# huj31415/nbody3d-webgpu

Hardware: AMD Instinct MI355X
Metric: pair-interactions/s (higher is better)
Workload: dtype f32; 1 GPU; N=262144 Plummer sphere, dt=1e-3, G=1, eps2=1e-4, i-sharded over 1 GPU(s); n=262144, kernel_variant=f32pk_symw_ipl16_j1_w2048_r32t128, parallelism=1gpu

## Files before the change

nbody3d-webgpu_amd/csrc/kernels/symmetric.hip.h:

```cpp
#pragma once

namespace nb {

template <typename T> struct SymRowT { T x, y, z; };
using SymRow = SymRowT<float>;

constexpr uint32_t kFlushSteps = 4096;

template <int NG>
__device__ __forceinline__ void flush_resident_sums(float (*hi)[64], const int lane, const bool flushed, nb_f2 (&ax)[NG], nb_f2 (&ay)[NG], nb_f2 (&az)[NG])
{
    if (flushed) {
#pragma unroll
        for (int c = 0; c < NG; ++c) {
            hi[6 * c + 0][lane] += ax[c].x; hi[6 * c + 1][lane] += ay[c].x; hi[6 * c + 2][lane] += az[c].x;
            hi[6 * c + 3][lane] += ax[c].y; hi[6 * c + 4][lane] += ay[c].y; hi[6 * c + 5][lane] += az[c].y;
        }
    } else {
#pragma unroll
        for (int c = 0; c < NG; ++c) {
            hi[6 * c + 0][lane] = ax[c].x; hi[6 * c + 1][lane] = ay[c].x; hi[6 * c + 2][lane] = az[c].x;
            hi[6 * c + 3][lane] = ax[c].y; hi[6 * c + 4][lane] = ay[c].y; hi[6 * c + 5][lane] = az[c].y;
        }
    }
// ... 95 lines not shown
                    for (int c = 0; c < 4; ++c) si[c] = pm * r[c];
#pragma unroll
                    for (int c = 0; c < 4; ++c) sj[c] = mi[c0g + c] * r[c];
#pragma unroll
                    for (int c = 0; c < 4; ++c) ax[c0g + c] = __builtin_elementwise_fma(si[c], dx[c], ax[c0g + c]);
#pragma unroll
                    for (int c = 0; c < 4; ++c) ay[c0g + c] = __builtin_elementwise_fma(si[c], dy[c], ay[c0g + c]);
#pragma unroll
                    for (int c = 0; c < 4; ++c) az[c0g + c] = __builtin_elementwise_fma(si[c], dz[c], az[c0g + c]);
#pragma unroll
                    for (int c = 0; c < 4; ++c) bx[u] = __builtin_elementwise_fma(-sj[c], dx[c], bx[u]);
#pragma unroll
                    for (int c = 0; c < 4; ++c) by[u] = __builtin_elementwise_fma(-sj[c], dy[c], by[u]);
#pragma unroll
                    for (int c = 0; c < 4; ++c) bz[u] = __builtin_elementwise_fma(-sj[c], dz[c], bz[u]);
                }
            }
#pragma unroll
            for (int u = 0; u < J; ++u) {
                tx[u] = wave_rot1(tx[u]); ty[u] = wave_rot1(ty[u]); tz[u] = wave_rot1(tz[u]); tm[u] = wave_rot1(tm[u]);
                bx[u] = nb_f2{wave_rot1(bx[u].x), wave_rot1(bx[u].y)};
                by[u] = nb_f2{wave_rot1(by[u].x), wave_rot1(by[u].y)};
                bz[u] = nb_f2{wave_rot1(bz[u].x), wave_rot1(bz[u].y)};
            }
        }
        if (sym) {
            SymRow* out = partial + (size_t)(pl.t_layer0 + d) * pl.np + tstart + lane;
            if constexpr (WS == 1) {
#pragma unroll
                for (int u = 0; u < J; ++u) out[u * 64] = SymRow{bx[u].x + bx[u].y, by[u].x + by[u].y, bz[u].x + bz[u].y};
            } else {
                const int buf = done++ & 1;
#pragma unroll
                for (int u = 0; u < J; ++u) {
                    red[buf][w][3 * u + 0][lane] = bx[u].x + bx[u].y;
                    red[buf][w][3 * u + 1][lane] = by[u].x + by[u].y;
                    red[buf][w][3 * u + 2][lane] = bz[u].x + bz[u].y;
                }
                __syncthreads();
                if (w == done % WS) {
#pragma unroll
                    for (int u = 0; u < J; ++u) {
                        float sx = red[buf][0][3 * u + 0][lane], sy = red[buf][0][3 * u + 1][lane], sz = red[buf][0][3 * u + 2][lane];
#pragma unroll
                        for (int ww = 1; ww < WS; ++ww) { sx += red[buf][ww][3 * u + 0][lane]; sy += red[buf][ww][3 * u + 1][lane]; sz += red[buf][ww][3 * u + 2][lane]; }
                        out[u * 64] = SymRow{sx, sy, sz};
                    }
                }
            }
        }
    }
    SymRow* out = partial + (size_t)(pl.r_layer0 + q) * pl.np + (size_t)g * S + w * RB + lane;
#pragma unroll
    for (int c = 0; c < NG; ++c) {
        out[(2 * c) * 64] = SymRow{ax[c].x, ay[c].x, az[c].x};
        out[(2 * c + 1) * 64] = SymRow{ax[c].y, ay[c].y, az[c].y};
    }
}

struct SymWK { uint32_t np, nsb, W, total_hi, total_lo, n_hi, zc, ups, r_layer0, t_layer0; };
#define SYMW_PLAN_PARAMS const uint32_t W_, const uint32_t ups_, const uint32_t nsb_, const uint32_t zc_, const uint32_t r_layer0_, const uint32_t t_layer0_
typedef uint32_t nb_u4 __attribute__((ext_vector_type(4)));
template <int TAIL>
__device__ __forceinline__ void symw_record_and_tail(const uint32_t* rec_at, nb_u4& rec, uint32_t (&tail)[TAIL])
{
    static_assert(TAIL == 1 || TAIL == 4, "f32: eps2; f64: G, eps2");
    constexpr int kTailOffset = 4 * 8 + 6 * 4;
    if constexpr (TAIL == 1) {
        asm volatile("s_load_dwordx4 %0, %2, 0x0\n\ts_load_dword %1, %3, %4\n\ts_waitcnt lgkmcnt(0)"
                     : "=&s"(rec), "=&s"(tail[0]) : "s"(rec_at), "s"(__builtin_amdgcn_kernarg_segment_ptr()), "n"(kTailOffset) : "memory");
    } else {
        nb_u4 t;
        asm volatile("s_load_dwordx4 %0, %2, 0x0\n\ts_load_dwordx4 %1, %3, %4\n\ts_waitcnt lgkmcnt(0)"
                     : "=&s"(rec), "=&s"(t) : "s"(rec_at), "s"(__builtin_amdgcn_kernarg_segment_ptr()), "n"(kTailOffset) : "memory");
        tail[0] = t.x; tail[1] = t.y; tail[2] = t.z; tail[3] = t.w;
    }
}

__device__ __forceinline__ SymWK symw_plan_words(uint32_t S, uint32_t cps, uint32_t W, uint32_t ups, uint32_t nsb, uint32_t zc, uint32_t r_layer0, uint32_t t_layer0)
{
    const uint32_t H = (nsb - 1u) >> 1, n_hi = (nsb & 1u) ? 0u : nsb >> 1;
    const uint32_t total_lo = (H + 1u) * cps + zc, total_hi = total_lo + (n_hi ? cps : 0u);
    return SymWK{(nsb + (zc ? 1u : 0u)) * S, nsb, W, total_hi, total_lo, n_hi, zc, ups, r_layer0, t_layer0};
}

template <int NG, int J, bool PAIR>
__device__ __forceinline__ void symw_sweeps(const uint32_t* __restrict__ gtab, const float4* __restrict__ bodies, SymRow* __restrict__ partial, SymRow* __restrict__ spill,
                                            SYMW_PLAN_PARAMS, uint32_t* __restrict__ queue, const uint32_t npieces, const uint32_t pieces_off)
{
    static_assert(!PAIR || J == 1, "paired sweeps: one traveler per lane and sweep");
    constexpr uint32_t S = 128u * NG;
    constexpr int GW = NG < 4 ? NG : 4;
    constexpr uint32_t CH = 64u * J;
    constexpr uint32_t CPS = S / CH;
    const SymWK pl = symw_plan_words(S, CPS, W_, ups_, nsb_, zc_, r_layer0_, t_layer0_);
    const int lane = threadIdx.x & 63, wi = threadIdx.x >> 6;
    const uint32_t w = __builtin_amdgcn_readfirstlane(blockIdx.x * 4u + wi);
    const bool active = w < pl.W;
    NB_STAMP(0);
    __shared__ float red[4][6 * NG][64];
    __shared__ uint32_t fin[4];
    const uint32_t ups = pl.ups, ush = (uint32_t)__builtin_ctz(ups), ustep = 64u >> ush,
                   tab1 = 2u * (pl.np / S);
    nb_u4 rec;
    uint32_t tail[1];
    symw_record_and_tail(gtab + tab1 + 4u * (active ? w : 0u), rec, tail);
    const float eps2 = __builtin_bit_cast(float, tail[0]);
    const nb_f2 e2 = nb_f2{eps2, eps2};
    const uint32_t first_lo = pl.n_hi * pl.total_hi, first_z = first_lo + (pl.nsb - pl.n_hi) * pl.total_lo;
    const uint32_t slot = rec.w;
    NB_STAMP_LIGHT(1);
    bool first_part = true;

    auto run = [&](uint32_t u, const uint32_t uend, const uint32_t piece_layer) -> uint32_t {
        uint32_t gfin = ~0u;
        while (u < uend) {
            const uint32_t p = u >> ush;
            uint32_t g, k, total;
            if (p < first_lo) { g = p / pl.total_hi; k = p - g * pl.total_hi; total = pl.total_hi; }
            else if (p < first_z) { const uint32_t r = p - first_lo; g = pl.n_hi + r / pl.total_lo; k = r - (g - pl.n_hi) * pl.total_lo; total = pl.total_lo; }
            else { g = pl.nsb; k = p - first_z; total = pl.zc; }
            const uint32_t ring = g < pl.nsb ? total - CPS - pl.zc : 0u;
            const uint32_t both_end = g < pl.nsb ? ring + pl.zc : 0u;
            uint32_t ug_end = (p - k + total) * ups;
            if (ug_end > uend) ug_end = uend;

            nb_f2 xi[NG], yi[NG], zi[NG], mi[NG], ax[NG], ay[NG], az[NG];
            {
                const float4* rb = bodies + (size_t)g * S + lane;
#pragma unroll
                for (int c = 0; c < NG; ++c) {
                    const float4 b0 = ld4(rb + (2 * c) * 64), b1 = ld4(rb + (2 * c + 1) * 64);
                    xi[c] = nb_f2{b0.x, b1.x}; yi[c] = nb_f2{b0.y, b1.y}; zi[c] = nb_f2{b0.z, b1.z}; mi[c] = nb_f2{b0.w, b1.w};
                    ax[c] = nb_f2{0, 0}; ay[c] = nb_f2{0, 0}; az[c] = nb_f2{0, 0};
                }
            }
            uint32_t since = 0;
            bool flushed = false;
            while (u < ug_end) {
                const uint32_t q0 = u & (ups - 1u);
                bool pair = false;
                if constexpr (PAIR) pair = q0 == 0u && ug_end - u >= 2u * ups && k + 1u < both_end;
                uint32_t nun = ups - q0;
                if (nun > ug_end - u) nun = ug_end - u;
                const uint32_t s0 = q0 * ustep, s1 = s0 + nun * ustep;
                u += pair ? 2u * ups : nun;
                if (since >= kFlushSteps) {
                    flush_resident_sums<NG>(red[wi], lane, flushed, ax, ay, az);
                    flushed = true;
                    since = 0;
                }
                since += pair ? 128u : s1 - s0;
                const bool sym = k < both_end, zsweep = k >= ring && sym;
                const uint32_t d = k / CPS;
                uint32_t tb = g + 1 + d;
                if (tb >= pl.nsb) tb -= pl.nsb;
                const uint32_t tstart = k < ring ? tb * S + (k % CPS) * CH : zsweep ? pl.nsb * S + (k - ring) * CH : g * S + (k - both_end) * CH;
                const uint32_t zrow = g * pl.zc + (k - ring);
                ++k;
                if constexpr (PAIR) {
                    if (pair) {
                        const bool zsweep1 = k >= ring;
                        const uint32_t d1 = k / CPS;
                        uint32_t tb1 = g + 1 + d1;
                        if (tb1 >= pl.nsb) tb1 -= pl.nsb;
                        const uint32_t tstart1 = zsweep1 ? pl.nsb * S + (k - ring) * CH : tb1 * S + (k % CPS) * CH;
// ... 319 lines not shown
                                uu[c] = nb_fma(t3 * e, 1.5, t3);
                            }
#pragma unroll
                            for (int c = 0; c < GW; ++c) {
                                const double si = tm * uu[c];
                                ax[c0g + c] = nb_fma(si, dx[c], ax[c0g + c]); ay[c0g + c] = nb_fma(si, dy[c], ay[c0g + c]); az[c0g + c] = nb_fma(si, dz[c], az[c0g + c]);
                                if constexpr (BOTH) {
                                    const double sj = mi[c0g + c] * uu[c];
                                    bx = nb_fma(-sj, dx[c], bx); by = nb_fma(-sj, dy[c], by); bz = nb_fma(-sj, dz[c], bz);
                                }
                            }
                        }
                        tx = wave_rot1(tx); ty = wave_rot1(ty); tz = wave_rot1(tz); tm = wave_rot1(tm);
                        if constexpr (BOTH) { bx = wave_rot1(bx); by = wave_rot1(by); bz = wave_rot1(bz); }
                    }
                };
                if (sym) steps(std::true_type{}); else steps(std::false_type{});
                if (sym) {
                    SymRowT<double>* out = (s0 != 0 ? spill + (size_t)slot * CH : zsweep ? spill + (size_t)zrow * CH : partial + (size_t)(pl.t_layer0 + d) * pl.np + tstart)
                                           + (((uint32_t)lane - s1) & 63u);
                    *out = SymRowT<double>{bx, by, bz};
                }
            }
            if (u >= uend && piece_layer != ~0u) {
                SymRowT<double>* out = partial + (size_t)(pl.r_layer0 + piece_layer) * pl.np + (size_t)g * S + lane;
#pragma unroll
                for (int c = 0; c < IPL; ++c) out[c * 64] = SymRowT<double>{ax[c], ay[c], az[c]};
                return g;
            }
            if (u >= uend) {
                gfin = g;
#pragma unroll
                for (int c = 0; c < IPL; ++c) { red[wi][3 * c + 0][lane] = ax[c]; red[wi][3 * c + 1][lane] = ay[c]; red[wi][3 * c + 2][lane] = az[c]; }
                break;
            }
            SymRowT<double>* out = partial + (size_t)(pl.r_layer0 + gtab[2 * g + 1] - 1u) * pl.np + (size_t)g * S + lane;
#pragma unroll
            for (int c = 0; c < IPL; ++c) out[c * 64] = SymRowT<double>{ax[c], ay[c], az[c]};
        }
        return gfin;
    };
    const uint32_t gfin = run(active ? rec.x : 0u, active ? rec.y : 0u, ~0u);
    if (lane == 0) fin[wi] = gfin;
    __syncthreads();
    if (gfin != ~0u) {
        int members = 0, mine = 0;
#pragma unroll
        for (int j = 0; j < 4; ++j) {
            const bool same = fin[j] == gfin;
            members += same;
            mine += same && j < wi;
        }
        SymRowT<double>* out = partial + (size_t)(pl.r_layer0 + rec.z) * pl.np + (size_t)gfin * S + lane;
        for (int r = mine; r < IPL; r += members) {
            double sx = 0, sy = 0, sz = 0;
#pragma unroll
            for (int j = 0; j < 4; ++j)
                if (fin[j] == gfin) { sx += red[j][3 * r + 0][lane]; sy += red[j][3 * r + 1][lane]; sz += red[j][3 * r + 2][lane]; }
            out[r * 64] = SymRowT<double>{sx, sy, sz};
        }
    }
    if (npieces) {
        for (;;) {
            uint32_t id = 0;
            if (lane == 0) id = __hip_atomic_fetch_add(queue, 1u, __ATOMIC_RELAXED, __HIP_MEMORY_SCOPE_AGENT);
            id = __builtin_amdgcn_readfirstlane(id);
            if (id >= npieces) break;
            const uint32_t pu = gtab[pieces_off + 2u * id], ll = gtab[pieces_off + 2u * id + 1u];
            (void)run(pu, pu + (ll >> 16), ll & 0xffffu);
        }
    }
}

__device__ __forceinline__ uint32_t rank_find(const uint32_t* __restrict__ prefix, uint32_t ng, uint32_t p)
{
    uint32_t lo = 0, hi = ng;
    while (hi - lo > 1) {
        const uint32_t mid = (lo + hi) >> 1;
        if (prefix[mid] <= p) lo = mid; else hi = mid;
    }
    return lo;
}

template <int NG>
__global__ __launch_bounds__(256) __attribute__((amdgpu_waves_per_eu(NG > 4 ? 2 : 4, NG > 4 ? 2 : 4)))
void nb_force_symw_rank(const float4* __restrict__ bodies, SymRow* __restrict__ partial, const uint32_t* __restrict__ tab, const SymRankPlan pl,
                        const uint32_t n, const float eps2, const uint32_t wave0, const uint32_t wave_end, SymRow* __restrict__ spill,
                        const uint32_t k_lo, const uint32_t k_hi, const uint32_t d0)
{
    constexpr uint32_t S = 128u * NG, CPS = S / 64u;
    constexpr int GW = NG < 4 ? NG : 4;
    const int lane = threadIdx.x & 63;
    const uint32_t w = wave0 + __builtin_amdgcn_readfirstlane(blockIdx.x * 4u + (threadIdx.x >> 6));
    if (w >= wave_end) return;
    const bool phase_b = w >= pl.WA;
    const uint32_t wl = phase_b ? w - pl.WA : w, Lp = phase_b ? pl.LB : pl.LA, Wp = phase_b ? pl.WB : pl.WA;
    const uint32_t ng = pl.g1 - pl.g0;
    const size_t lstride = (size_t)ng * S;
    const uint32_t* __restrict__ prefix = tab + 4 * pl.nsb + (phase_b ? ng + 1 : 0);
    const uint32_t ups = pl.ups, ustep = 64u / ups;
    const uint64_t Lu = (uint64_t)Lp * ups;
    uint32_t u = (uint32_t)(((uint64_t)wl * Lu) / Wp);
    const uint32_t uend = (uint32_t)(((uint64_t)(wl + 1) * Lu) / Wp);
    const nb_f2 e2 = nb_f2{eps2, eps2};
    __shared__ float hi[4][6 * NG][64];
    const int wi = threadIdx.x >> 6;
    while (u < uend) {
        const uint32_t ps = u / ups;
        const uint32_t gi = rank_find(prefix, ng, ps), g = pl.g0 + gi;
        uint32_t j = ps - prefix[gi];
        uint32_t ug_end = prefix[gi + 1] * ups;
        if (ug_end > uend) ug_end = uend;
        const uint32_t total = g < pl.n_hi ? pl.total_hi : pl.total_lo, ring = total - CPS;
        uint32_t a = (pl.g1 - 1 - g) * CPS;
        if (a > ring) a = ring;
        const uint32_t a_lo = a < k_lo ? a : k_lo, a_len = (a < k_hi ? a : k_hi) - a_lo;
        uint32_t b_lo = a > k_lo ? a : k_lo;
        if (b_lo > ring) b_lo = ring;

        nb_f2 xi[NG], yi[NG], zi[NG], mi[NG], ax[NG], ay[NG], az[NG];
        {
            const float4* rb = bodies + (size_t)g * S + lane;
#pragma unroll
            for (int c = 0; c < NG; ++c) {
                const float4 b0 = ld4(rb + (2 * c) * 64), b1 = ld4(rb + (2 * c + 1) * 64);
                xi[c] = nb_f2{b0.x, b1.x}; yi[c] = nb_f2{b0.y, b1.y}; zi[c] = nb_f2{b0.z, b1.z}; mi[c] = nb_f2{b0.w, b1.w};
                ax[c] = nb_f2{0, 0}; ay[c] = nb_f2{0, 0}; az[c] = nb_f2{0, 0};
            }
        }
        uint32_t since = 0;
        bool flushed = false;
        while (u < ug_end) {
            const uint32_t q0 = u % ups;
            uint32_t nun = ups - q0;
            if (nun > ug_end - u) nun = ug_end - u;
            const uint32_t s0 = q0 * ustep, s1 = s0 + nun * ustep;
            u += nun;
            const uint32_t k = phase_b ? b_lo + j : (j < a_len ? a_lo + j : ring + (j - a_len));
            ++j;
            const bool sym = k < ring;
            const uint32_t d = k / CPS;
            uint32_t tb = g + 1 + d;
            if (tb >= pl.nsb) tb -= pl.nsb;
            const uint32_t tstart = sym ? tb * S + (k % CPS) * 64u : g * S + (k - ring) * 64u;
            if (tstart >= n) continue;
            if (since >= kFlushSteps) {
                flush_resident_sums<NG>(hi[wi], lane, flushed, ax, ay, az);
                flushed = true;
                since = 0;
            }
            since += s1 - s0;
            const float4 t = ld4(bodies + tstart + (((uint32_t)lane - s0) & 63u));
            float tx = t.x, ty = t.y, tz = t.z, tm = t.w;
            nb_f2 bx = nb_f2{0, 0}, by = nb_f2{0, 0}, bz = nb_f2{0, 0};
            for (uint32_t st = s0; st < s1; ++st) {
                const nb_f2 px = nb_f2{tx, tx}, py = nb_f2{ty, ty}, pz = nb_f2{tz, tz}, pm = nb_f2{tm, tm};
#pragma unroll
                for (int c0g = 0; c0g < NG; c0g += GW) {
                    nb_f2 dx[GW], dy[GW], dz[GW], d2[GW], r[GW], si[GW], sj[GW];
#pragma unroll
                    for (int c = 0; c < GW; ++c) dx[c] = px - xi[c0g + c];
#pragma unroll
                    for (int c = 0; c < GW; ++c) dy[c] = py - yi[c0g + c];
#pragma unroll
                    for (int c = 0; c < GW; ++c) dz[c] = pz - zi[c0g + c];
#pragma unroll
                    for (int c = 0; c < GW; ++c) d2[c] = __builtin_elementwise_fma(dx[c], dx[c], e2);
#pragma unroll
                    for (int c = 0; c < GW; ++c) d2[c] = __builtin_elementwise_fma(dy[c], dy[c], d2[c]);
#pragma unroll
                    for (int c = 0; c < GW; ++c) d2[c] = __builtin_elementwise_fma(dz[c], dz[c], d2[c]);
#pragma unroll
                    for (int c = 0; c < GW; ++c) r[c] = d2[c] * d2[c];
#pragma unroll
                    for (int c = 0; c < GW; ++c) r[c] = r[c] * d2[c];
#pragma unroll
                    for (int c = 0; c < GW; ++c) r[c] = nb_f2{nb_rsq(r[c].x), nb_rsq(r[c].y)};
#pragma unroll
                    for (int c = 0; c < GW; ++c) si[c] = pm * r[c];
#pragma unroll
                    for (int c = 0; c < GW; ++c) sj[c] = mi[c0g + c] * r[c];
#pragma unroll
                    for (int c = 0; c < GW; ++c) ax[c0g + c] = __builtin_elementwise_fma(si[c], dx[c], ax[c0g + c]);
#pragma unroll
                    for (int c = 0; c < GW; ++c) ay[c0g + c] = __builtin_elementwise_fma(si[c], dy[c], ay[c0g + c]);
#pragma unroll
                    for (int c = 0; c < GW; ++c) az[c0g + c] = __builtin_elementwise_fma(si[c], dz[c], az[c0g + c]);
#pragma unroll
                    for (int c = 0; c < GW; ++c) bx = __builtin_elementwise_fma(-sj[c], dx[c], bx);
#pragma unroll
                    for (int c = 0; c < GW; ++c) by = __builtin_elementwise_fma(-sj[c], dy[c], by);
#pragma unroll
                    for (int c = 0; c < GW; ++c) bz = __builtin_elementwise_fma(-sj[c], dz[c], bz);
                }
                tx = wave_rot1(tx); ty = wave_rot1(ty); tz = wave_rot1(tz); tm = wave_rot1(tm);
                bx = nb_f2{wave_rot1(bx.x), wave_rot1(bx.y)};
                by = nb_f2{wave_rot1(by.x), wave_rot1(by.y)};
                bz = nb_f2{wave_rot1(bz.x), wave_rot1(bz.y)};
            }
            if (sym) {
                SymRow* out = (s0 == 0 ? partial + (size_t)(pl.t_layer0 + d - d0) * lstride + (size_t)gi * S + (k % CPS) * 64u : spill + (size_t)w * 64u) + (((uint32_t)lane - s1) & 63u);
                *out = SymRow{bx.x + bx.y, by.x + by.y, bz.x + bz.y};
            }
        }
        const uint32_t* gt = tab + 4 * g;
        SymRow* out = partial + (size_t)(phase_b ? pl.rb_layer0 + (wl - gt[2]) : pl.r_layer0 + (wl - gt[0])) * lstride + (size_t)gi * S + lane;
#pragma unroll
        for (int c = 0; c < NG; ++c) {
            if (flushed) {
                ax[c].x += hi[wi][6 * c + 0][lane]; ay[c].x += hi[wi][6 * c + 1][lane]; az[c].x += hi[wi][6 * c + 2][lane];
                ax[c].y += hi[wi][6 * c + 3][lane]; ay[c].y += hi[wi][6 * c + 4][lane]; az[c].y += hi[wi][6 * c + 5][lane];
            }
            out[(2 * c) * 64] = SymRow{ax[c].x, ay[c].x, az[c].x};
            out[(2 * c + 1) * 64] = SymRow{ax[c].y, ay[c].y, az[c].y};
        }
    }
}

template <int IPL>
__global__ __launch_bounds__(256) __attribute__((amdgpu_waves_per_eu(2, 2)))
void nb_force_symw64_rank(const double4* __restrict__ bodies, SymRowT<double>* __restrict__ partial, const uint32_t* __restrict__ tab,
                          const SymRankPlan pl, const uint32_t n, const double G, const double eps2, const uint32_t wave0, const uint32_t wave_end,
                          SymRowT<double>* __restrict__ spill, const uint32_t k_lo, const uint32_t k_hi, const uint32_t d0)
{
    constexpr uint32_t S = 64u * IPL, CPS = S / 64u;
    constexpr int GW = 4;
    const int lane = threadIdx.x & 63;
    const uint32_t w = wave0 + __builtin_amdgcn_readfirstlane(blockIdx.x * 4u + (threadIdx.x >> 6));
    if (w >= wave_end) return;
    const bool phase_b = w >= pl.WA;
    const uint32_t wl = phase_b ? w - pl.WA : w, Lp = phase_b ? pl.LB : pl.LA, Wp = phase_b ? pl.WB : pl.WA;
    const uint32_t ng = pl.g1 - pl.g0;
    const size_t lstride = (size_t)ng * S;
    const uint32_t* __restrict__ prefix = tab + 4 * pl.nsb + (phase_b ? ng + 1 : 0);
    const uint32_t ups = pl.ups, ustep = 64u / ups;
    const uint64_t Lu = (uint64_t)Lp * ups;
    uint32_t u = (uint32_t)(((uint64_t)wl * Lu) / Wp);
    const uint32_t uend = (uint32_t)(((uint64_t)(wl + 1) * Lu) / Wp);
    while (u < uend) {
        const uint32_t ps = u / ups;
        const uint32_t gi = rank_find(prefix, ng, ps), g = pl.g0 + gi;
        uint32_t j = ps - prefix[gi];
        uint32_t ug_end = prefix[gi + 1] * ups;
        if (ug_end > uend) ug_end = uend;
        const uint32_t total = g < pl.n_hi ? pl.total_hi : pl.total_lo, ring = total - CPS;
        uint32_t a = (pl.g1 - 1 - g) * CPS;
        if (a > ring) a = ring;
        const uint32_t a_lo = a < k_lo ? a : k_lo, a_len = (a < k_hi ? a : k_hi) - a_lo;
        uint32_t b_lo = a > k_lo ? a : k_lo;
        if (b_lo > ring) b_lo = ring;
        double xi[IPL], yi[IPL], zi[IPL], mi[IPL], ax[IPL], ay[IPL], az[IPL];
#pragma unroll
        for (int c = 0; c < IPL; ++c) {
            const double4 b = ld4(bodies + (size_t)g * S + c * 64 + lane);
            xi[c] = b.x; yi[c] = b.y; zi[c] = b.z; mi[c] = b.w * G;
            ax[c] = 0; ay[c] = 0; az[c] = 0;
        }
        while (u < ug_end) {
            const uint32_t q0 = u % ups;
            uint32_t nun = ups - q0;
            if (nun > ug_end - u) nun = ug_end - u;
            const uint32_t s0 = q0 * ustep, s1 = s0 + nun * ustep;
            u += nun;
            const uint32_t k = phase_b ? b_lo + j : (j < a_len ? a_lo + j : ring + (j - a_len));
            ++j;
            const bool sym = k < ring;
            const uint32_t d = k / CPS;
            uint32_t tb = g + 1 + d;
            if (tb >= pl.nsb) tb -= pl.nsb;
            const uint32_t tstart = sym ? tb * S + (k % CPS) * 64u : g * S + (k - ring) * 64u;
            if (tstart >= n) continue;
            const double4 t = ld4(bodies + tstart + (((uint32_t)lane - s0) & 63u));
            double tx = t.x, ty = t.y, tz = t.z, tm = t.w * G, bx = 0, by = 0, bz = 0;
            for (uint32_t st = s0; st < s1; ++st) {
#pragma unroll
                for (int c0g = 0; c0g < IPL; c0g += GW) {
                    double dx[GW], dy[GW], dz[GW], d2[GW], y[GW], uu[GW];
#pragma unroll
                    for (int c = 0; c < GW; ++c) dx[c] = tx - xi[c0g + c];
#pragma unroll
                    for (int c = 0; c < GW; ++c) dy[c] = ty - yi[c0g + c];
#pragma unroll
                    for (int c = 0; c < GW; ++c) dz[c] = tz - zi[c0g + c];
#pragma unroll
                    for (int c = 0; c < GW; ++c) d2[c] = nb_fma(dz[c], dz[c], nb_fma(dy[c], dy[c], nb_fma(dx[c], dx[c], eps2)));
// ... 247 lines not shown
```

nbody3d-webgpu_amd/csrc/nb_engine.hip:

```cpp
#include "nb_internal.h"
#include "nb_kernels.hip.h"
#include "../../include/nbody3d_hip_plan.h"

#include <hip/hip_ext.h>

#include <algorithm>
#include <cmath>
#include <cstdio>
#include <cstdlib>
#include <cstring>
#include <new>
#include <type_traits>

namespace {
thread_local std::string g_create_error = "";
}

namespace nbi {
int fail(nb_sim* s, int code, const std::string& msg)
{
    if (s) s->err = msg; else g_create_error = msg;
    return code;
}
void set_create_error(const std::string& msg) { g_create_error = msg; }
// ... 4 lines not shown

using nbi::fail;

#define NB_HIP(s, call)                                                                                   \
    do {                                                                                                  \
        hipError_t e_ = (call);                                                                           \
        if (e_ != hipSuccess)                                                                             \
            return fail((s), NB_ERR_HIP, std::string(#call) + ": " + hipGetErrorString(e_));              \
    } while (0)

using namespace nbp;

#define NB_LS_CASES(F, NG, TL, ls)                                      \
    switch (ls) {                                                        \
        case 1: return (const void*)&nb::F<NG, 1, TL>;                   \
        case 2: return (const void*)&nb::F<NG, 2, TL>;                   \
        case 4: return (const void*)&nb::F<NG, 4, TL>;                   \
        case 8: return (const void*)&nb::F<NG, 8, TL>;                   \
        case 16: return (const void*)&nb::F<NG, 16, TL>;                 \
        case 32: return (const void*)&nb::F<NG, 32, TL>;                 \
        case 64: return (const void*)&nb::F<NG, 64, TL>;                 \
        default: return nullptr;                                         \
    }
#define NB_LS_CASES_T4(F, NG, ls)                                       \
    switch (ls) {                                                        \
        case 16: return (const void*)&nb::F<NG, 16, 4>;                  \
        case 32: return (const void*)&nb::F<NG, 32, 4>;                  \
        case 64: return (const void*)&nb::F<NG, 64, 4>;                  \
        default: return nullptr;                                         \
    }
#define NB_LS_CASES_T8(F, NG, ls)                                       \
    switch (ls) {                                                        \
        case 32: return (const void*)&nb::F<NG, 32, 8>;                  \
        case 64: return (const void*)&nb::F<NG, 64, 8>;                  \
        default: return nullptr;                                         \
    }
#define NB_PK_TABLE(NAME, F)                                            \
    const void* NAME(int ng, int ls, int tl)                            \
    {                                                                    \
        if (tl == 8) {           \
            if (ng == 1) { NB_LS_CASES_T8(F, 1, ls) }                    \
            if (ng == 2) { NB_LS_CASES_T8(F, 2, ls) }                    \
            if (ng == 4) { NB_LS_CASES_T8(F, 4, ls) }                    \
        }                                                                \
        if (tl == 1) {                                                   \
            if (ng == 1) { NB_LS_CASES(F, 1, 1, ls) }                    \
            if (ng == 2) { NB_LS_CASES(F, 2, 1, ls) }                    \
            if (ng == 4) { NB_LS_CASES(F, 4, 1, ls) }                    \
        } else if (tl == 4) {                                            \
            if (ng == 1) { NB_LS_CASES_T4(F, 1, ls) }                    \
            if (ng == 2) { NB_LS_CASES_T4(F, 2, ls) }                    \
            if (ng == 4) { NB_LS_CASES_T4(F, 4, ls) }                    \
        }                                                                \
        return nullptr;                                                  \
    }
NB_PK_TABLE(pk_force_kernel, nb_force_pk)
NB_PK_TABLE(pk_fused_kernel, nb_step_fused)

template <typename T>
const void* scalar_kernel(int ipl, int ls)
{
    if (ls == 1) {
        if (ipl == 1) return (const void*)&nb::nb_force<T, 1, 1>;
        if (ipl == 2) return (const void*)&nb::nb_force<T, 2, 1>;
        if (ipl == 4) return (const void*)&nb::nb_force<T, 4, 1>;
        return nullptr;
    }
    if (ipl != 1) return nullptr;
    if (ls == 4) return (const void*)&nb::nb_force<T, 1, 4>;
    if (ls == 16) return (const void*)&nb::nb_force<T, 1, 16>;
    if (ls == 64) return (const void*)&nb::nb_force<T, 1, 64>;
    return nullptr;
}

const void* sgpr_kernel(int ipl, int ws)
{
    if (ipl == 4 && ws == 5) return (const void*)&nb::nb_force_pk_sgpr<2, 4, true>;
    if (ipl == 4) return ws == 4 ? (const void*)&nb::nb_force_pk_sgpr<2, 4> : (const void*)&nb::nb_force_pk_sgpr<2, 1>;
    if (ipl == 8 && ws == 5) return (const void*)&nb::nb_force_pk_sgpr<4, 4, true>;
    if (ipl == 8) return ws == 4 ? (const void*)&nb::nb_force_pk_sgpr<4, 4> : (const void*)&nb::nb_force_pk_sgpr<4, 1>;
    return nullptr;
}

const void* rank_kernel_of(bool f64, int ipl)
{
    if (f64) return ipl == 8 ? (const void*)&nb::nb_force_symw64_rank<8> : nullptr;
    return ipl == 16 ? (const void*)&nb::nb_force_symw_rank<8> : ipl == 8 ? (const void*)&nb::nb_force_symw_rank<4> : nullptr;
}

const void* kernel_of(bool f64, const Shape& sh, bool single_sweeps = false)
{
    switch (sh.kind) {
        case kScalar: return f64 ? scalar_kernel<double>(sh.ipl, sh.ls) : scalar_kernel<float>(sh.ipl, sh.ls);
        case kPkLds: return f64 || (sh.ipl & 1) ? nullptr : pk_force_kernel(sh.ipl / 2, sh.ls, sh.x);
        case kFused: return f64 || (sh.ipl & 1) ? nullptr : pk_fused_kernel(sh.ipl / 2, sh.ls, sh.x);
        case kPkSgpr: return f64 || sh.ls != 1 || !(sh.x == 1 || sh.x == 4 || sh.x == 5) ? nullptr : sgpr_kernel(sh.ipl, sh.x);
        case kDirect:
            if (f64 || sh.ipl != 2 || sh.ls != 64) return nullptr;
            return sh.x == 1 ? (const void*)&nb::nb_step_direct<16> : sh.x == 2 ? (const void*)&nb::nb_step_direct<32> : nullptr;
        case kSym:
            if (sh.ls != 1) return nullptr;
            if (f64) return sh.ipl == 8 && sh.x == 3 ? (const void*)&nb::nb_force_symw64<8> : nullptr;
            if (sh.x == 4) return sh.ipl == 8 ? (const void*)&nb::nb_force_sym<4, 4, 2> : nullptr;
            if (sh.ipl == 4) return sh.x == 3 ? (const void*)&nb::nb_force_symw<2, 1> : nullptr;
            if (sh.ipl == 8 && sh.x == 3) return single_sweeps ? (const void*)&nb::nb_force_symw<4, 1> : (const void*)&nb::nb_force_symw_pairs<4>;
            if (sh.ipl == 16 && sh.x == 3) return single_sweeps ? (const void*)&nb::nb_force_symw<8, 1> : (const void*)&nb::nb_force_symw_pairs<8>;
            if (sh.ipl == 8) return sh.x == 1 ? (const void*)&nb::nb_force_symw<4, 2> : nullptr;
            if (sh.ipl == 16) return sh.x == 1 ? (const void*)&nb::nb_force_symw<8, 2> : nullptr;
            return nullptr;
        case kJpk:
            if (f64 || sh.ipl != 1 || sh.ls != 1) return nullptr;
            return sh.x == 4 ? (const void*)&nb::nb_step_jpk<4> : sh.x == 8 ? (const void*)&nb::nb_step_jpk<8>
                   : sh.x == 6 ? (const void*)&nb::nb_step_jpk<16> : nullptr;
        default: return nullptr;
    }
}

void plan_handle(nb_sim* s, const nb_config& cfg, int n_cu, double clock_hz, double device_mem)
{
    PlanInput in;
    if (device_mem > 0) in.device_mem = device_mem;
    in.n = s->n; in.sb = s->sb; in.sc = s->sc; in.f64 = s->f64; in.cfg = cfg; in.n_cu = n_cu; in.clock_hz = clock_hz;
    if (!s->no_device)
        in.occupancy = [f64 = s->f64](const Shape& sh, int block) {
            int occ = 0;
            const void* fn = kernel_of(f64, sh);
            if (!fn || hipOccupancyMaxActiveBlocksPerMultiprocessor(&occ, fn, block, 0) != hipSuccess) { (void)hipGetLastError(); return 0; }
            return occ;
        };
    LaunchPlan p = plan_launch(in);
    s->ipl = p.ipl; s->ls = p.ls; s->ws = p.ws; s->tl = p.tl;
    s->packed = p.packed; s->sgpr = p.sgpr; s->fused = p.fused; s->direct = p.direct; s->jpk = p.jpk; s->swap_acc = p.swap_acc;
    s->jsplit = p.jsplit; s->j_per_split = p.j_per_split; s->junits = p.junits; s->own_split0 = p.own_split0; s->own_splits = p.own_splits;
    s->sym = p.sym; s->symw = p.symw; s->sym_rank = p.sym_rank;
    s->sym_np = p.sym_np; s->sym_layers = p.sym_layers; s->sym_g0 = p.sym_g0; s->sym_g1 = p.sym_g1;
    static_assert(sizeof(s->sym_plan) == sizeof(p.sym_plan), "nb_sim::sym_plan mirrors LaunchPlan::sym_plan");
    memcpy(s->sym_plan, p.sym_plan, sizeof s->sym_plan);
    static_assert(sizeof(s->sym_rank_plan) == sizeof(p.sym_rank_plan), "nb_sim::sym_rank_plan mirrors LaunchPlan::sym_rank_plan");
    memcpy(s->sym_rank_plan, p.sym_rank_plan, sizeof s->sym_rank_plan);
    s->sym_passes = std::move(p.sym_passes);
    s->sym_local = p.sym_local;
    s->sym_tab_host = std::move(p.sym_tab_host);
    s->sym_spill_rows = p.sym_spill_rows;
    s->sym_pieces = p.sym_pieces;
    s->variant = std::move(p.variant);
}

Shape shape_of(const nb_sim* s)
{
    if (s->sym) return {kSym, s->ipl, 1, s->ws};
    if (s->jpk) return {kJpk, 1, 1, s->ws};
    if (s->direct) return {kDirect, s->ipl, s->ls, s->tl};
    if (s->fused) return {kFused, s->ipl, s->ls, s->tl};
    if (s->sgpr) return {kPkSgpr, s->ipl, 1, s->ws};
    if (s->packed) return {kPkLds, s->ipl, s->ls, s->tl};
    return {kScalar, s->ipl, s->ls, 1};
}

size_t sym_layer_rows(const nb_sim* s) { return s->sym_rank ? (size_t)(s->sym_g1 - s->sym_g0) * ipb_of(shape_of(s)) : (size_t)s->sym_np; }

bool streams_gm(const nb_sim* s) { return !s->f64 && s->packed && !s->jpk; }
bool gm_active(const nb_sim* s) { return streams_gm(s) && (float)s->G != 1.0f; }
const void* jstream(const nb_sim* s, int k) { return gm_active(s) ? s->gm[k] : s->bodies[k]; }

int ensure_gm(nb_sim* s)
{
    if (!gm_active(s)) { s->gm_ok = false; return NB_OK; }
    const size_t bytes = (size_t)16 * (s->sym ? s->sym_np : s->n);
    for (int k = 0; k < (s->fused ? 2 : 1); ++k)
        if (!s->gm[k]) {
            NB_HIP(s, hipMalloc(&s->gm[k], bytes));
            if (s->sym) NB_HIP(s, hipMemsetAsync(s->gm[k], 0, bytes, s->stream));
        }
    if (s->gm_ok && s->gm_G == s->G) return NB_OK;
    const float4* b = (const float4*)s->bodies[s->cur];
    float4* g = (float4*)s->gm[s->cur];
    uint32_t n = s->n;
    float G = (float)s->G;
    void* args[] = {&b, &g, &n, &G};
    NB_HIP(s, hipLaunchKernel((const void*)&nb::nb_gm_pack<0>, dim3(ceil_div(n, nb::kBlock)), dim3(nb::kBlock), args, 0, s->stream));
    s->gm_ok = true; s->gm_G = s->G;
    return NB_OK;
}

void launch_kernel(const void* fn, dim3 grid, dim3 block, void** args, hipStream_t stream, hipEvent_t t0, hipEvent_t t1)
{
    if (t0 || t1) (void)hipExtLaunchKernel(fn, grid, block, args, 0, stream, t0, t1, 0);
    else (void)hipLaunchKernel(fn, grid, block, args, 0, stream);
}

template <typename T>
void launch_force(nb_sim* s, int part = 0, hipEvent_t t0 = nullptr, hipEvent_t t1 = nullptr)
{
    using V4 = typename nb::vec4<T>::type;
    const Shape sh = shape_of(s);
    if (s->sym_rank) {
        const nbp::LaunchPlan::SymPass& ps = s->sym_passes[s->sym_pass];
        nb::SymRankPlan rp;
        memcpy(&rp, ps.plan, sizeof rp);
        uint32_t w0 = part == 2 ? rp.WA : 0u, w1 = part == 1 ? rp.WA : rp.WA + rp.WB;
        if (w1 <= w0) return;
        const void* b = jstream(s, s->cur);
        void* p = s->partial;
        const uint32_t* tab = s->sym_tab + ps.tab_off;
        uint32_t n = s->n, k_lo = ps.k_lo, k_hi = ps.k_hi, d0 = ps.d0;
        void* sp = s->sym_spill;
        if (s->f64) {
            double G = s->G, e2 = s->eps2;
            void* args[] = {&b, &p, &tab, &rp, &n, &G, &e2, &w0, &w1, &sp, &k_lo, &k_hi, &d0};
            launch_kernel(rank_kernel_of(true, sh.ipl), dim3(ceil_div(w1 - w0, 4u)), dim3(256), args, s->stream, t0, t1);
        } else {
            float e2 = (float)s->eps2;
            void* args[] = {&b, &p, &tab, &rp, &n, &e2, &w0, &w1, &sp, &k_lo, &k_hi, &d0};
            launch_kernel(rank_kernel_of(false, sh.ipl), dim3(ceil_div(w1 - w0, 4u)), dim3(256), args, s->stream, t0, t1);
        }
        return;
    }
    if (s->symw) {
        nb::SymWPlan pl;
        memcpy(&pl, s->sym_plan, sizeof pl);
        const void* b = jstream(s, s->cur);
        void* p = s->partial;
        const uint32_t* tab = s->sym_tab;
        void* sp = s->sym_spill;
        uint32_t* queue = s->sym_queue;
        uint32_t npieces = s->sym_pieces, pieces_off = 2u * (pl.np / ipb_of(sh)) + 4u * pl.W;
        if (npieces) (void)hipMemsetAsync(queue, 0, sizeof(uint32_t), s->stream);
        if (s->f64) {
            double G = s->G, e2 = s->eps2;
            void* args[] = {&tab, &b, &p, &sp, &pl.W, &pl.ups, &pl.nsb, &pl.zc, &pl.r_layer0, &pl.t_layer0, &G, &e2, &queue, &npieces, &pieces_off};
            launch_kernel(kernel_of(true, sh), dim3(ceil_div(pl.W, 4u)), dim3(256), args, s->stream, t0, t1);
        } else {
            float e2 = (float)s->eps2;
            void* args[] = {&tab, &b, &p, &sp, &pl.W, &pl.ups, &pl.nsb, &pl.zc, &pl.r_layer0, &pl.t_layer0, &e2, &queue, &npieces, &pieces_off};
            launch_kernel(kernel_of(false, sh, s->single_sweeps), dim3(ceil_div(pl.W, 4u)), dim3(256), args, s->stream, t0, t1);
        }
        return;
    }
    if (s->sym) {
        nb::SymPlan pl;
        memcpy(&pl, s->sym_plan, sizeof pl);
        const float4* b = (const float4*)jstream(s, s->cur);
        nb::SymRow* p = (nb::SymRow*)s->partial;
        float e2 = (float)s->eps2;
        uint32_t n = s->n;
        void* args[] = {&b, &p, &pl, &n, &e2};
        launch_kernel(kernel_of(false, sh), dim3(pl.nsb * pl.q), dim3(64 * sh.x), args, s->stream, t0, t1);
        return;
    }
    nb::SplitWindow win{0, 0xffffffffu, 0};
    uint32_t ny = s->jsplit;
    if (part == 1) { win.base = s->own_split0; ny = s->own_splits; }
    else if (part == 2) { win.hole_begin = s->own_split0; win.hole_count = s->own_splits; ny = s->jsplit - s->own_splits; }
    if (ny == 0) return;
    dim3 grid(ceil_div(s->sc, ipb_of(sh)), ny), block(nb::kBlock);
    const V4* b = (const V4*)jstream(s, s->cur);
    V4* p = (V4*)s->partial;
    T G = (T)s->G, e2 = (T)s->eps2;
    uint32_t n = s->n, sb = s->sb, sc = s->sc, jps = s->j_per_split;
    const V4* zr = (const V4*)s->zero_row;
    void* args[] = {&b, &p, &n, &sb, &sc, &G, &e2, &jps, &win, &zr};
    launch_kernel(kernel_of(s->f64, sh), grid, block, args, s->stream, t0, t1);
}

void ensure_pairs(nb_sim* s)
{
    if (!s->jpk || (s->pairs_ok && s->pairs_G == s->G)) return;
    const float4* b = (const float4*)s->bodies[s->cur];
    float4* p = (float4*)s->pairs[s->cur];
    uint32_t n = s->n;
    float G = (float)s->G;
    void* args[] = {&b, &p, &n, &G};
    (void)hipLaunchKernel((const void*)&nb::nb_pairs_pack<0>, dim3(ceil_div(ceil_div(n, 2u), nb::kBlock)), dim3(nb::kBlock), args, 0, s->stream);
    s->pairs_ok = true; s->pairs_G = s->G;
}

void launch_jpk(nb_sim* s, hipEvent_t t0, hipEvent_t t1)
{
    const Shape sh = shape_of(s);
    dim3 grid(ceil_div(s->n, 64u), s->jsplit), block(64 * jpk_ws(sh.x));
    const float4 *bin = (const float4*)s->bodies[s->cur], *pin = (const float4*)s->pairs[s->cur];
    float4 *bout = (float4*)s->bodies[s->cur ^ 1], *pout = (float4*)s->pairs[s->cur ^ 1];
    float4 *v = (float4*)s->vel, *a = (float4*)s->acc, *part = (float4*)s->jpartial;
    uint32_t* tk = s->tickets;
    uint32_t n = s->n, upw = s->junits, poison = (s->poison ? 1u : 0u) | (s->jpk_fenced ? 2u : 0u);
    float G = (float)s->G, e2 = (float)s->eps2, dt = (float)s->dt;
    void* args[] = {&bin, &pin, &bout, &pout, &v, &a, &part, &tk, &n, &upw, &poison, &G, &e2, &dt};
    launch_kernel(kernel_of(false, sh), grid, block, args, s->stream, t0, t1);
    s->cur ^= 1;
}

void launch_fused(nb_sim* s, hipEvent_t t0 = nullptr, hipEvent_t t1 = nullptr)
{
    if (s->jpk) { ensure_pairs(s); launch_jpk(s, t0, t1); return; }
    const Shape sh = shape_of(s);
    dim3 grid(ceil_div(s->n, ipb_of(sh))), block(nb::kBlock);
    const float4 *bin = (const float4*)s->bodies[s->cur], *jin = (const float4*)jstream(s, s->cur);
// ... 1512 lines not shown
```

Measured before the change: 6684 billion pair-interactions/s.

## Pair two traveler chunks per sweep in rank symmetric kernel

Adds a paired-sweep path to the rank-scheduled symmetric f32 kernel. When a full aligned unit pair of symmetric chunks is available, it carries two traveler chunks per lane, one in each half of the packed float2, so each packed instruction covers two travelers instead of duplicating a single traveler. It also specializes non-symmetric (diagonal) chunks to skip the reaction-force accumulation and rotation. The aim is better packed-math utilization and fewer rotations per interaction, at the cost of higher register pressure (waves_per_eu minimum lowered to 2 for the paired variant) and more complex indexing.

```diff
diff --git a/nbody3d-webgpu_amd/csrc/kernels/symmetric.hip.h b/nbody3d-webgpu_amd/csrc/kernels/symmetric.hip.h
--- a/nbody3d-webgpu_amd/csrc/kernels/symmetric.hip.h
+++ b/nbody3d-webgpu_amd/csrc/kernels/symmetric.hip.h
@@ -201,6 +201,131 @@
     const uint32_t H = (nsb - 1u) >> 1, n_hi = (nsb & 1u) ? 0u : nsb >> 1;
     const uint32_t total_lo = (H + 1u) * cps + zc, total_hi = total_lo + (n_hi ? cps : 0u);
     return SymWK{(nsb + (zc ? 1u : 0u)) * S, nsb, W, total_hi, total_lo, n_hi, zc, ups, r_layer0, t_layer0};
+}
+
+template <int NG>
+__device__ __forceinline__ void symw_pair_steps(const nb_f2 (&xi)[NG], const nb_f2 (&yi)[NG], const nb_f2 (&zi)[NG], const nb_f2 (&mi)[NG],
+                                                nb_f2 (&ax)[NG], nb_f2 (&ay)[NG], nb_f2 (&az)[NG], const nb_f2 e2,
+                                                nb_f2& tx, nb_f2& ty, nb_f2& tz, nb_f2& tm,
+                                                float& bx0, float& bx1, float& by0, float& by1, float& bz0, float& bz1)
+{
+    constexpr int GW = NG < 4 ? NG : 4;
+    for (uint32_t st = 0; st < 64u; ++st) {
+        nb_f2 sx = nb_f2{0, 0}, sy = nb_f2{0, 0}, sz = nb_f2{0, 0};
+#pragma unroll
+        for (int c0g = 0; c0g < NG; c0g += GW) {
+#pragma unroll
+            for (int f = 0; f < 2; ++f) {
+                nb_f2 dx[GW], dy[GW], dz[GW], d2[GW], r[GW], si[GW], sj[GW];
+#pragma unroll
+                for (int c = 0; c < GW; ++c) dx[c] = symw_sub(f, tx, xi[c0g + c]);
+#pragma unroll
+                for (int c = 0; c < GW; ++c) dy[c] = symw_sub(f, ty, yi[c0g + c]);
+#pragma unroll
+                for (int c = 0; c < GW; ++c) dz[c] = symw_sub(f, tz, zi[c0g + c]);
+#pragma unroll
+                for (int c = 0; c < GW; ++c) d2[c] = __builtin_elementwise_fma(dx[c], dx[c], e2);
+#pragma unroll
+                for (int c = 0; c < GW; ++c) d2[c] = __builtin_elementwise_fma(dy[c], dy[c], d2[c]);
+#pragma unroll
+                for (int c = 0; c < GW; ++c) d2[c] = __builtin_elementwise_fma(dz[c], dz[c], d2[c]);
+#pragma unroll
+                for (int c = 0; c < GW; ++c) r[c] = d2[c] * d2[c];
+#pragma unroll
+                for (int c = 0; c < GW; ++c) r[c] = r[c] * d2[c];
+#pragma unroll
+                for (int c = 0; c < GW; ++c) r[c] = nb_f2{nb_rsq(r[c].x), nb_rsq(r[c].y)};
+#pragma unroll
+                for (int c = 0; c < GW; ++c) si[c] = symw_mul(f, tm, r[c]);
+#pragma unroll
+                for (int c = 0; c < GW; ++c) sj[c] = mi[c0g + c] * r[c];
+#pragma unroll
+                for (int c = 0; c < GW; ++c) ax[c0g + c] = __builtin_elementwise_fma(si[c], dx[c], ax[c0g + c]);
+#pragma unroll
+                for (int c = 0; c < GW; ++c) ay[c0g + c] = __builtin_elementwise_fma(si[c], dy[c], ay[c0g + c]);
+#pragma unroll
+                for (int c = 0; c < GW; ++c) az[c0g + c] = __builtin_elementwise_fma(si[c], dz[c], az[c0g + c]);
+#pragma unroll
+                for (int c = 0; c < GW; ++c) sx = symw_fnma(f, sj[c], dx[c], sx);
+#pragma unroll
+                for (int c = 0; c < GW; ++c) sy = symw_fnma(f, sj[c], dy[c], sy);
+#pragma unroll
+                for (int c = 0; c < GW; ++c) sz = symw_fnma(f, sj[c], dz[c], sz);
+            }
+        }
+        tx = nb_f2{wave_rot1(tx.x), wave_rot1(tx.y)}; ty = nb_f2{wave_rot1(ty.x), wave_rot1(ty.y)};
+        tz = nb_f2{wave_rot1(tz.x), wave_rot1(tz.y)}; tm = nb_f2{wave_rot1(tm.x), wave_rot1(tm.y)};
+        wave_rot1_add(bx0, sx.x); wave_rot1_add(bx1, sx.y); wave_rot1_add(by0, sy.x); wave_rot1_add(by1, sy.y);
+        wave_rot1_add(bz0, sz.x); wave_rot1_add(bz1, sz.y);
+        __builtin_amdgcn_sched_barrier(0);
+    }
+}
+
+template <int NG, int J, bool BOTH>
+__device__ __forceinline__ void symw_steps(const uint32_t s0, const uint32_t s1,
+                                           const nb_f2 (&xi)[NG], const nb_f2 (&yi)[NG], const nb_f2 (&zi)[NG], const nb_f2 (&mi)[NG],
+                                           nb_f2 (&ax)[NG], nb_f2 (&ay)[NG], nb_f2 (&az)[NG], const nb_f2 e2,
+                                           float (&tx)[J], float (&ty)[J], float (&tz)[J], float (&tm)[J], nb_f2 (&bx)[J], nb_f2 (&by)[J], nb_f2 (&bz)[J])
+{
+    constexpr int GW = NG < 4 ? NG : 4;
+    for (uint32_t st = s0; st < s1; ++st) {
+#pragma unroll
+        for (int uu = 0; uu < J; ++uu) {
+            const nb_f2 px = nb_f2{tx[uu], tx[uu]}, py = nb_f2{ty[uu], ty[uu]}, pz = nb_f2{tz[uu], tz[uu]}, pm = nb_f2{tm[uu], tm[uu]};
+#pragma unroll
+            for (int c0g = 0; c0g < NG; c0g += GW) {
+                nb_f2 dx[GW], dy[GW], dz[GW], d2[GW], r[GW], si[GW], sj[GW];
+#pragma unroll
+                for (int c = 0; c < GW; ++c) dx[c] = px - xi[c0g + c];
+#pragma unroll
+                for (int c = 0; c < GW; ++c) dy[c] = py - yi[c0g + c];
+#pragma unroll
+                for (int c = 0; c < GW; ++c) dz[c] = pz - zi[c0g + c];
+#pragma unroll
+                for (int c = 0; c < GW; ++c) d2[c] = __builtin_elementwise_fma(dx[c], dx[c], e2);
+#pragma unroll
+                for (int c = 0; c < GW; ++c) d2[c] = __builtin_elementwise_fma(dy[c], dy[c], d2[c]);
+#pragma unroll
+                for (int c = 0; c < GW; ++c) d2[c] = __builtin_elementwise_fma(dz[c], dz[c], d2[c]);
+#pragma unroll
+                for (int c = 0; c < GW; ++c) r[c] = d2[c] * d2[c];
+#pragma unroll
+                for (int c = 0; c < GW; ++c) r[c] = r[c] * d2[c];
+#pragma unroll
+                for (int c = 0; c < GW; ++c) r[c] = nb_f2{nb_rsq(r[c].x), nb_rsq(r[c].y)};
+#pragma unroll
+                for (int c = 0; c < GW; ++c) si[c] = pm * r[c];
+                if constexpr (BOTH) {
+#pragma unroll
+                    for (int c = 0; c < GW; ++c) sj[c] = mi[c0g + c] * r[c];
+                }
+#pragma unroll
+                for (int c = 0; c < GW; ++c) ax[c0g + c] = __builtin_elementwise_fma(si[c], dx[c], ax[c0g + c]);
+#pragma unroll
+                for (int c = 0; c < GW; ++c) ay[c0g + c] = __builtin_elementwise_fma(si[c], dy[c], ay[c0g + c]);
+#pragma unroll
+                for (int c = 0; c < GW; ++c) az[c0g + c] = __builtin_elementwise_fma(si[c], dz[c], az[c0g + c]);
+                if constexpr (BOTH) {
+#pragma unroll
+                    for (int c = 0; c < GW; ++c) bx[uu] = __builtin_elementwise_fma(-sj[c], dx[c], bx[uu]);
+#pragma unroll
+                    for (int c = 0; c < GW; ++c) by[uu] = __builtin_elementwise_fma(-sj[c], dy[c], by[uu]);
+#pragma unroll
+                    for (int c = 0; c < GW; ++c) bz[uu] = __builtin_elementwise_fma(-sj[c], dz[c], bz[uu]);
+                }
+            }
+        }
+#pragma unroll
+        for (int uu = 0; uu < J; ++uu) {
+            tx[uu] = wave_rot1(tx[uu]); ty[uu] = wave_rot1(ty[uu]); tz[uu] = wave_rot1(tz[uu]); tm[uu] = wave_rot1(tm[uu]);
+            if constexpr (BOTH) {
+                bx[uu] = nb_f2{wave_rot1(bx[uu].x), wave_rot1(bx[uu].y)};
+                by[uu] = nb_f2{wave_rot1(by[uu].x), wave_rot1(by[uu].y)};
+                bz[uu] = nb_f2{wave_rot1(bz[uu].x), wave_rot1(bz[uu].y)};
+            }
+        }
+        if constexpr (!BOTH) __builtin_amdgcn_sched_barrier(0);
+    }
 }
 
 template <int NG, int J, bool PAIR>
@@ -686,14 +811,13 @@
     return lo;
 }
 
-template <int NG>
-__global__ __launch_bounds__(256) __attribute__((amdgpu_waves_per_eu(NG > 4 ? 2 : 4, NG > 4 ? 2 : 4)))
+template <int NG, bool PAIR>
+__global__ __launch_bounds__(256) __attribute__((amdgpu_waves_per_eu(NG > 4 || PAIR ? 2 : 4, NG > 4 ? 2 : 4)))
 void nb_force_symw_rank(const float4* __restrict__ bodies, SymRow* __restrict__ partial, const uint32_t* __restrict__ tab, const SymRankPlan pl,
                         const uint32_t n, const float eps2, const uint32_t wave0, const uint32_t wave_end, SymRow* __restrict__ spill,
                         const uint32_t k_lo, const uint32_t k_hi, const uint32_t d0)
 {
     constexpr uint32_t S = 128u * NG, CPS = S / 64u;
-    constexpr int GW = NG < 4 ? NG : 4;
     const int lane = threadIdx.x & 63;
     const uint32_t w = wave0 + __builtin_amdgcn_readfirstlane(blockIdx.x * 4u + (threadIdx.x >> 6));
     if (w >= wave_end) return;
@@ -739,72 +863,58 @@
             uint32_t nun = ups - q0;
             if (nun > ug_end - u) nun = ug_end - u;
             const uint32_t s0 = q0 * ustep, s1 = s0 + nun * ustep;
-            u += nun;
             const uint32_t k = phase_b ? b_lo + j : (j < a_len ? a_lo + j : ring + (j - a_len));
-            ++j;
             const bool sym = k < ring;
             const uint32_t d = k / CPS;
             uint32_t tb = g + 1 + d;
             if (tb >= pl.nsb) tb -= pl.nsb;
             const uint32_t tstart = sym ? tb * S + (k % CPS) * 64u : g * S + (k - ring) * 64u;
+            bool pair = false;
+            uint32_t d1 = 0, tstart1 = 0;
+            if constexpr (PAIR) {
+                if (q0 == 0u && ug_end - u >= 2u * ups && (phase_b ? k + 1u < ring : j + 1u < a_len)) {
+                    d1 = (k + 1u) / CPS;
+                    uint32_t tb1 = g + 1 + d1;
+                    if (tb1 >= pl.nsb) tb1 -= pl.nsb;
+                    tstart1 = tb1 * S + ((k + 1u) % CPS) * 64u;
+                    pair = tstart < n && tstart1 < n;
+                }
+            }
+            u += pair ? 2u * ups : nun;
+            j += pair ? 2u : 1u;
             if (tstart >= n) continue;
             if (since >= kFlushSteps) {
                 flush_resident_sums<NG>(hi[wi], lane, flushed, ax, ay, az);
                 flushed = true;
                 since = 0;
             }
-            since += s1 - s0;
+            since += pair ? 128u : s1 - s0;
+            if constexpr (PAIR) {
+                if (pair) {
+                    const float4 t0 = ld4(bodies + tstart + lane), t1 = ld4(bodies + tstart1 + lane);
+                    nb_f2 tx = nb_f2{t0.x, t1.x}, ty = nb_f2{t0.y, t1.y}, tz = nb_f2{t0.z, t1.z}, tm = nb_f2{t0.w, t1.w};
+                    float bx0 = 0, bx1 = 0, by0 = 0, by1 = 0, bz0 = 0, bz1 = 0;
+                    symw_pair_steps<NG>(xi, yi, zi, mi, ax, ay, az, e2, tx, ty, tz, tm, bx0, bx1, by0, by1, bz0, bz1);
+                    const uint32_t home = ((uint32_t)lane + 1u) & 63u;
+                    SymRow* out0 = partial + (size_t)(pl.t_layer0 + d - d0) * lstride + (size_t)gi * S + (k % CPS) * 64u + home;
+                    SymRow* out1 = partial + (size_t)(pl.t_layer0 + d1 - d0) * lstride + (size_t)gi * S + ((k + 1u) % CPS) * 64u + home;
+                    *out0 = SymRow{bx0, by0, bz0};
+                    *out1 = SymRow{bx1, by1, bz1};
+                    continue;
+                }
+            }
             const float4 t = ld4(bodies + tstart + (((uint32_t)lane - s0) & 63u));
-            float tx = t.x, ty = t.y, tz = t.z, tm = t.w;
-            nb_f2 bx = nb_f2{0, 0}, by = nb_f2{0, 0}, bz = nb_f2{0, 0};
-            for (uint32_t st = s0; st < s1; ++st) {
-                const nb_f2 px = nb_f2{tx, tx}, py = nb_f2{ty, ty}, pz = nb_f2{tz, tz}, pm = nb_f2{tm, tm};
-#pragma unroll
-                for (int c0g = 0; c0g < NG; c0g += GW) {
-                    nb_f2 dx[GW], dy[GW], dz[GW], d2[GW], r[GW], si[GW], sj[GW];
-#pragma unroll
-                    for (int c = 0; c < GW; ++c) dx[c] = px - xi[c0g + c];
-#pragma unroll
-                    for (int c = 0; c < GW; ++c) dy[c] = py - yi[c0g + c];
-#pragma unroll
-                    for (int c = 0; c < GW; ++c) dz[c] = pz - zi[c0g + c];
-#pragma unroll
-                    for (int c = 0; c < GW; ++c) d2[c] = __builtin_elementwise_fma(dx[c], dx[c], e2);
-#pragma unroll
-                    for (int c = 0; c < GW; ++c) d2[c] = __builtin_elementwise_fma(dy[c], dy[c], d2[c]);
-#pragma unroll
-                    for (int c = 0; c < GW; ++c) d2[c] = __builtin_elementwise_fma(dz[c], dz[c], d2[c]);
-#pragma unroll
-                    for (int c = 0; c < GW; ++c) r[c] = d2[c] * d2[c];
-#pragma unroll
-                    for (int c = 0; c < GW; ++c) r[c] = r[c] * d2[c];
-#pragma unroll
-                    for (int c = 0; c < GW; ++c) r[c] = nb_f2{nb_rsq(r[c].x), nb_rsq(r[c].y)};
-#pragma unroll
-                    for (int c = 0; c < GW; ++c) si[c] = pm * r[c];
-#pragma unroll
-                    for (int c = 0; c < GW; ++c) sj[c] = mi[c0g + c] * r[c];
-#pragma unroll
-                    for (int c = 0; c < GW; ++c) ax[c0g + c] = __builtin_elementwise_fma(si[c], dx[c], ax[c0g + c]);
-#pragma unroll
-                    for (int c = 0; c < GW; ++c) ay[c0g + c] = __builtin_elementwise_fma(si[c], dy[c], ay[c0g + c]);
-#pragma unroll
-                    for (int c = 0; c < GW; ++c) az[c0g + c] = __builtin_elementwise_fma(si[c], dz[c], az[c0g + c]);
-#pragma unroll
-                    for (int c = 0; c < GW; ++c) bx = __builtin_elementwise_fma(-sj[c], dx[c], bx);
-#pragma unroll
-                    for (int c = 0; c < GW; ++c) by = __builtin_elementwise_fma(-sj[c], dy[c], by);
-#pragma unroll
-                    for (int c = 0; c < GW; ++c) bz = __builtin_elementwise_fma(-sj[c], dz[c], bz);
-                }
-                tx = wave_rot1(tx); ty = wave_rot1(ty); tz = wave_rot1(tz); tm = wave_rot1(tm);
-                bx = nb_f2{wave_rot1(bx.x), wave_rot1(bx.y)};
-                by = nb_f2{wave_rot1(by.x), wave_rot1(by.y)};
-                bz = nb_f2{wave_rot1(bz.x), wave_rot1(bz.y)};
-            }
-            if (sym) {
-                SymRow* out = (s0 == 0 ? partial + (size_t)(pl.t_layer0 + d - d0) * lstride + (size_t)gi * S + (k % CPS) * 64u : spill + (size_t)w * 64u) + (((uint32_t)lane - s1) & 63u);
-                *out = SymRow{bx.x + bx.y, by.x + by.y, bz.x + bz.y};
+            float tx[1] = {t.x}, ty[1] = {t.y}, tz[1] = {t.z}, tm[1] = {t.w};
+            if (sym || !PAIR) {
+                nb_f2 bx[1] = {nb_f2{0, 0}}, by[1] = {nb_f2{0, 0}}, bz[1] = {nb_f2{0, 0}};
+                symw_steps<NG, 1, true>(s0, s1, xi, yi, zi, mi, ax, ay, az, e2, tx, ty, tz, tm, bx, by, bz);
+                if (sym) {
+                    SymRow* out = (s0 == 0 ? partial + (size_t)(pl.t_layer0 + d - d0) * lstride + (size_t)gi * S + (k % CPS) * 64u : spill + (size_t)w * 64u) + (((uint32_t)lane - s1) & 63u);
+                    *out = SymRow{bx[0].x + bx[0].y, by[0].x + by[0].y, bz[0].x + bz[0].y};
+                }
+            } else {
+                nb_f2 none[1];
+                symw_steps<NG, 1, false>(s0, s1, xi, yi, zi, mi, ax, ay, az, e2, tx, ty, tz, tm, none, none, none);
             }
         }
         const uint32_t* gt = tab + 4 * g;
diff --git a/nbody3d-webgpu_amd/csrc/nb_engine.hip b/nbody3d-webgpu_amd/csrc/nb_engine.hip
--- a/nbody3d-webgpu_amd/csrc/nb_engine.hip
+++ b/nbody3d-webgpu_amd/csrc/nb_engine.hip
@@ -110,10 +110,12 @@
     return nullptr;
 }
 
-const void* rank_kernel_of(bool f64, int ipl)
+const void* rank_kernel_of(bool f64, int ipl, bool single_sweeps = false)
 {
     if (f64) return ipl == 8 ? (const void*)&nb::nb_force_symw64_rank<8> : nullptr;
-    return ipl == 16 ? (const void*)&nb::nb_force_symw_rank<8> : ipl == 8 ? (const void*)&nb::nb_force_symw_rank<4> : nullptr;
+    if (ipl == 16) return single_sweeps ? (const void*)&nb::nb_force_symw_rank<8, false> : (const void*)&nb::nb_force_symw_rank<8, true>;
+    if (ipl == 8) return single_sweeps ? (const void*)&nb::nb_force_symw_rank<4, false> : (const void*)&nb::nb_force_symw_rank<4, true>;
+    return nullptr;
 }
 
 const void* kernel_of(bool f64, const Shape& sh, bool single_sweeps = false)
@@ -240,7 +242,7 @@
         } else {
             float e2 = (float)s->eps2;
             void* args[] = {&b, &p, &tab, &rp, &n, &e2, &w0, &w1, &sp, &k_lo, &k_hi, &d0};
-            launch_kernel(rank_kernel_of(false, sh.ipl), dim3(ceil_div(w1 - w0, 4u)), dim3(256), args, s->stream, t0, t1);
+            launch_kernel(rank_kernel_of(false, sh.ipl, s->single_sweeps), dim3(ceil_div(w1 - w0, 4u)), dim3(256), args, s->stream, t0, t1);
         }
         return;
     }
```

After: 6683 billion pair-interactions/s, median of 2. No clear change (-0.0%).
